# pyscf/pyscf

Hardware: NVIDIA H100
Metric: J/K Fock-build wall-s/iter (lower is better)
Workload: dtype f64

## Files before the change

### pyscf_b200/csrc/b200jk.cu

```cuda
#include "host_common.hpp"
#include "jk_classes.cuh"

namespace {

void ensure_workspace(b200jk_handle h, int n_dm)
{
    if ((size_t)n_dm <= h->ws_ndm) return;
    for (double** p : {&h->d_dm_sph, &h->d_out_sph, &h->d_dmj, &h->d_dmk, &h->d_vj, &h->d_vk}) { dev_free(*p); *p = nullptr; }
    size_t ns2 = (size_t)h->nsph * h->nsph, nc2 = (size_t)h->ncart * h->ncart;
    h->d_dm_sph = (double*)dev_alloc(ns2 * n_dm * 8);
    h->d_out_sph = (double*)dev_alloc(ns2 * n_dm * 8 * 2);
    h->d_dmj = (double*)dev_alloc(nc2 * n_dm * 8);
    h->d_dmk = (double*)dev_alloc(nc2 * n_dm * 8 * 2);
    h->d_vj = (double*)dev_alloc(nc2 * n_dm * 8);
    h->d_vk = (double*)dev_alloc(nc2 * n_dm * 8 * 2);
    h->ws_ndm = n_dm;
}

}

extern "C" const char* b200jk_version(void)
{
#ifdef B200JK_EMULATE
    return "b200jk 0.1 (CPU SIMT emulation — tests only)";
// ... 640 lines not shown
        d2h(w, dw, (size_t)count * n * 8, st);
#ifndef B200JK_EMULATE
        CK(cudaStreamSynchronize(st));
#endif
    } catch (std::exception& e) { set_err(h, e.what()); rc = 2; }
    for (void* p : tmp) dev_free(p);
    return rc;
}

extern "C" int b200jk_get_dm_cond_test(b200jk_handle h, double* dmc, int32_t* ao_off, int nsh)
{
    if (!h) return 1;
    try {
        if (!dmc || nsh != h->nsh) throw std::runtime_error("b200jk_get_dm_cond_test: nsh must be the number of device shells");
        if (!h->ws_ndm) throw std::runtime_error("b200jk_get_dm_cond_test: no b200jk_direct_jk call yet");
#ifndef B200JK_EMULATE
        CK(cudaSetDevice(h->device));
#endif
        d2h(dmc, h->d_dmc, (size_t)nsh * nsh * 8);
        dev_sync();
        if (ao_off)
            for (int i = 0; i < nsh; i++) ao_off[i] = h->sh[i].sph_off;
    } catch (std::exception& e) { set_err(h, e.what()); return 2; }
    return 0;
}

extern "C" int b200jk_get_stats(b200jk_handle h, b200jk_stats* out)
{
    if (!h || !out) return 1;
    *out = h->stats;
    return 0;
}

#ifndef B200JK_HAVE_DF
extern "C" int b200jk_df_build(b200jk_handle h, const int32_t*, int, const int32_t*, int, const double*, int, double, double)
{ set_err(h, "density-fitting path not built into this library"); return 3; }
extern "C" int b200jk_df_jk(b200jk_handle h, const double*, int, int, const double*, int, int, double*, double*)
{ set_err(h, "density-fitting path not built into this library"); return 3; }
extern "C" int b200jk_df_naux(b200jk_handle h, int*)
{ set_err(h, "density-fitting path not built into this library"); return 3; }
#endif
```

### pyscf_b200/csrc/jk_block.cuh

```cuda
#pragma once
#include "jk_core.cuh"

namespace b200jk {

constexpr int KCH_MAX = 512;
#ifndef B2_CTA_THREADS
#define B2_CTA_THREADS 192
#endif
#ifndef B2_SMEM_CAP
#define B2_SMEM_CAP 0
#endif

struct KParams {
    const ShellPair* bra_pairs; int nbra;
    const ShellPair* ket_pairs; int nket;
    int same_class;
    const PrimPair* prims;
    RysTables tb;
    double omega, tol;
    const double* dmc; int nsh;
    const double* dmj; const double* dmk;
    double* vj; double* vk;
    int n, n_dm_j, n_dm_k;
    int kchunk;
    int bra_nprim_max, ket_nprim_max;
    int shard_rank, shard_world;
    int pslice;
    unsigned long long* counters;
};

constexpr int pow2ceil(int x) { int p = 1; while (p < x) p *= 2; return p; }

#ifndef B2_PPW
#define B2_PPW 0
#endif

constexpr bool class_prefers_ppw(int li, int lj, int lk, int ll)
{
    return (li == 2 && lj == 2 && lk == 1 && ll == 1) || (li == 3 && lj == 3 && lk == 2 && ll == 0) || (li == 3 && lj == 2 && lk == 2 && ll == 0) ||
           (li == 2 && lj == 2 && lk == 2 && ll == 1) || (li == 2 && lj == 2 && lk == 2 && ll == 0) || (li == 3 && lj == 2 && lk == 1 && ll == 1);
}
template <class C>
struct GroupCfg {
    static constexpr int G = C::G;
    static constexpr bool PPW = (B2_PPW > 0 || (B2_PPW == 0 && class_prefers_ppw(C::LI, C::LJ, C::LK, C::LL))) && C::NP > 1 && C::NKL <= 32 && C::NP <= 8;
    static constexpr int GP = G <= 32 ? G : ((G + 31) / 32) * 32;
    static constexpr int GW = PPW ? C::NP : (GP + 31) / 32;
    static constexpr int TG = GW * 32;
    static constexpr int QPG = PPW ? 32 / C::NKL : (GP <= 32 ? 32 / GP : 1);
    static constexpr int NG0 = B2_CTA_THREADS / TG;
    static constexpr int NG1 = NG0 < 1 ? 1 : (NG0 > 8 ? 8 : NG0);
    static constexpr int NG2 = (NG1 * QPG > 64) ? ((64 / QPG) < 1 ? 1 : 64 / QPG) : NG1;
    static constexpr int NGC = B2_SMEM_CAP > 0 ? (int)(B2_SMEM_CAP / (QPG * sizeof(SlotSmem<C>))) : NG2;
    static constexpr int NG = NGC < 1 ? 1 : (NGC < NG2 ? NGC : NG2);
    static constexpr int NT = NG * TG;
    static constexpr int NSLOT = NG * QPG;
    static B2_HD bool decode(int lt, int& sl, int& g)
    {
        const int w = lt / 32, l = lt % 32;
        sl = l / C::NKL;
        g = w * C::NKL + l % C::NKL;
        if (sl >= QPG) { sl = 0; g = 0; return false; }
        return true;
    }
};

template <class C>
struct BlockSmem {
    SlotSmem<C> slot[GroupCfg<C>::NSLOT];
    BraInfo bra;
    PrimPair bprim[MAX_PRIM_PER_PAIR];
    unsigned long long mbar_bra;
    int klist[KCH_MAX];
    int nk;
    int next;
    int gbase[GroupCfg<C>::NG];
};

template <class C>
struct LaneCtx {
    ThreadCtx<C> t;
    double jij[C::NV];
    int grp, lt, slot, valid;
    int ibp, ikp;
    int sr;
};

#if defined(__CUDA_ARCH__)
#define B2_ALL_THREADS(tid) { const int tid = threadIdx.x;
#define B2_END }
#define B2_SYNC() __syncthreads()
#define B2_GROUP_LANES(lt) { const int lt = threadIdx.x % GroupCfg<C>::TG;
#define B2_CTX(tid) ctx
template <class C>
__device__ __forceinline__ void group_sync(int grp)
{
    if constexpr (GroupCfg<C>::GW == 1) __syncwarp();
    else asm volatile("bar.sync %0, %1;" ::"r"(grp + 1), "n"(GroupCfg<C>::TG) : "memory");
}
#else
#define B2_ALL_THREADS(tid) for (int tid = 0; tid < GroupCfg<C>::NT; tid++) {
#define B2_END }
#define B2_SYNC()
#define B2_GROUP_LANES(lt) for (int lt = 0; lt < GroupCfg<C>::TG; lt++) {
#define B2_CTX(tid) ctxs[tid]
template <class C>
inline void group_sync(int) {}
#endif

#if defined(__CUDA_ARCH__)
__device__ __forceinline__ void bulk_g2s(void* dst, const void* src, unsigned bytes, unsigned long long* bar)
{
    unsigned d = (unsigned)__cvta_generic_to_shared(dst), b = (unsigned)__cvta_generic_to_shared(bar);
    asm volatile("fence.proxy.async.shared::cta;" ::: "memory");
    asm volatile("mbarrier.arrive.expect_tx.shared::cta.b64 _, [%0], %1;" ::"r"(b), "r"(bytes) : "memory");
    asm volatile("cp.async.bulk.shared::cluster.global.mbarrier::complete_tx::bytes [%0], [%1], %2, [%3];"
                 ::"r"(d), "l"(src), "r"(bytes), "r"(b) : "memory");
}
__device__ __forceinline__ void bulk_wait(unsigned long long* bar, unsigned parity)
{
    unsigned b = (unsigned)__cvta_generic_to_shared(bar), ok;
    do {
        asm volatile("{\n\t.reg .pred p;\n\tmbarrier.try_wait.parity.shared::cta.b64 p, [%1], %2;\n\tselp.u32 %0, 1, 0, p;\n\t}\n"
                     : "=r"(ok) : "r"(b), "r"(parity) : "memory");
    } while (!ok);
}
#endif

template <class C, bool SR>
#ifdef __CUDACC__
__device__ __forceinline__
#else
inline
// ... 116 lines not shown

        for (int ip = 0; ip < npmax; ip++) {
            B2_GROUP_LANES(lt)
                LaneCtx<C>& L = B2_CTX(tid0 + lt);
                if (L.valid) {
                    SlotSmem<C>& s = sm.slot[L.slot];
                    if (s.active && L.ibp < nbp)
                        phase_roots<C>(s, L.t.g, sm.bprim[L.ibp], load_prim(P.prims + s.prim_off_k + L.ikp), P.tb,
                                       sr_op ? (L.sr ? -P.omega : 0.0) : P.omega, (sr_op && L.sr) ? -1.0 : 1.0);
                }
            B2_END
            group_sync<C>(grp);
            B2_GROUP_LANES(lt)
                LaneCtx<C>& L = B2_CTX(tid0 + lt);
                if (L.valid) {
                    SlotSmem<C>& s = sm.slot[L.slot];
                    if (s.active && L.ibp < nbp) phase_vrr<C>(s, L.t.g);
                }
            B2_END
            group_sync<C>(grp);
            B2_GROUP_LANES(lt)
                LaneCtx<C>& L = B2_CTX(tid0 + lt);
                if (L.valid) {
                    SlotSmem<C>& s = sm.slot[L.slot];
                    if (s.active && L.ibp < nbp) {
                        phase_accumulate<C>(s, L.t, sm.bra.ABx, sm.bra.ABy, sm.bra.ABz);
                        if (sr_op && !L.sr) L.sr = 1;
                        else { L.sr = 0; if (++L.ikp == s.nprim_k) { L.ikp = 0; L.ibp++; } }
                    }
                }
            B2_END
        }
        }
        B2_GROUP_LANES(lt)
            LaneCtx<C>& L = B2_CTX(tid0 + lt);
            if (L.valid) {
                SlotSmem<C>& s = sm.slot[L.slot];
                if (s.active) {
                    if (P.vj) phase_digest<C>(s, L.t, sm.bra.i0, sm.bra.j0, P.n, P.n_dm_j, P.dmj, nullptr, P.vj, nullptr,
                                              P.n_dm_j == 1 ? L.jij : nullptr);
                    if (P.vk) phase_digest<C>(s, L.t, sm.bra.i0, sm.bra.j0, P.n, P.n_dm_k, nullptr, P.dmk, nullptr, P.vk, nullptr);
                }
            }
        B2_END
        group_sync<C>(grp);
    }
}

template <class C, bool SR>
#ifdef __CUDACC__
__device__ __forceinline__
#else
inline
#endif
void jk_block(const KParams& P, int bx, int by, BlockSmem<C>& sm)
{
    using GC = GroupCfg<C>;
    const ShellPair& bpair = P.bra_pairs[bx];
    const int kmax = P.same_class ? (bx + 1) : P.nket;
    const int kbeg = by * P.kchunk;
    const int kend = (kbeg + P.kchunk < kmax) ? kbeg + P.kchunk : kmax;
    if (kbeg >= kend) return;
#if defined(__CUDA_ARCH__)
    LaneCtx<C> ctx;
#else
    LaneCtx<C>* ctxs = new LaneCtx<C>[GC::NT];
#endif

    B2_ALL_THREADS(tid)
        LaneCtx<C>& L = B2_CTX(tid);
        L.grp = tid / GC::TG;
        L.lt = tid % GC::TG;
        if constexpr (GC::PPW) {
            int sl, g;
            L.valid = GC::decode(L.lt, sl, g);
            L.slot = L.grp * GC::QPG + sl;
            thread_decode<C>(L.t, g);
// ... 33 lines not shown
        const int send = (sub + KCH_MAX < kend) ? sub + KCH_MAX : kend;
        if (sub > kbeg) {
            B2_SYNC();
            B2_ALL_THREADS(tid)
                if (tid == 0) { sm.nk = 0; sm.next = 0; }
            B2_END
            B2_SYNC();
        }
        B2_ALL_THREADS(tid)
            for (int kk = sub + tid; kk < send; kk += GC::NT) {
                const ShellPair& kp = P.ket_pairs[kk];
                bool keep = keep_quartet(bpair.q, kp.q, bpair.ish, bpair.jsh, kp.ish, kp.jsh, P.dmc, P.nsh, P.tol,
                                         P.vj != nullptr, P.vk != nullptr);
                if (keep) {
#if defined(__CUDA_ARCH__)
                    int pos = atomicAdd(&sm.nk, 1);
#else
                    int pos = sm.nk++;
#endif
                    sm.klist[pos] = kk;
                }
            }
        B2_END
        B2_SYNC();
        const int nk = sm.nk;
#if defined(__CUDA_ARCH__)
        if (P.counters && threadIdx.x == 0) {
            atomicAdd(&P.counters[0], (unsigned long long)nk);
            atomicAdd(&P.counters[1], (unsigned long long)(send - sub - nk));
        }
        group_proc<C, SR>(P, sm, threadIdx.x / GC::TG, nk, bx, ctx);
#else
        if (P.counters) { P.counters[0] += nk; P.counters[1] += send - sub - nk; }
        for (int grp = 0; grp < GC::NG; grp++) group_proc<C, SR>(P, sm, grp, nk, bx, ctxs);
#endif
    }

    if (P.vj && P.n_dm_j == 1) {
        B2_ALL_THREADS(tid)
            LaneCtx<C>& L = B2_CTX(tid);
            if (L.valid) {
                const int b0 = L.t.p * C::NJP;
                B2_UNROLL
                for (int bb = 0; bb < C::NJP; bb++) {
                    B2_UNROLL
                    for (int a = 0; a < C::NI; a++) {
                        double val = L.jij[bb * C::NI + a];
                        if (val != 0.0) red_add(&P.vj[(size_t)(sm.bra.i0 + a) * P.n + (sm.bra.j0 + b0 + bb)], val);
                    }
                }
            }
        B2_END
    }
#if !defined(__CUDA_ARCH__)
    delete[] ctxs;
#endif
}

}
```

### pyscf_b200/csrc/jk_core.cuh

```cuda
#pragma once
#include <math.h>
#include <stdint.h>

#ifdef __CUDACC__
#define B2_HD __host__ __device__ __forceinline__
#define B2_UNROLL _Pragma("unroll")
#define B2_NOUNROLL _Pragma("unroll 1")
#else
#define B2_HD inline __attribute__((always_inline))
#define B2_UNROLL
#define B2_NOUNROLL
#endif

namespace b200jk {

#ifndef __CUDACC__
inline double rsqrt(double x) { return 1.0 / sqrt(x); }
#endif

constexpr int LMAX = 4;
constexpr int RYS_NMAX = 9, RYS_DEG = 7, RYS_NINT = 320;
constexpr double RYS_H = 0.3125, RYS_XMAX = 100.0;
constexpr int RYS_ROW = 2 * (RYS_DEG + 1);
constexpr double PI_25_2 = 34.98683665524972497;
// ... 356 lines not shown

template <class C, int P>
struct PartDispatch {
    static B2_HD void run(int p, double* v, const double* gx, const double* gy, const double* gz)
    {
        if (p == P) accumulate_part<C, P>(v, gx, gy, gz);
        else PartDispatch<C, P + 1>::run(p, v, gx, gy, gz);
    }
};
template <class C>
struct PartDispatch<C, C::NP> {
    static B2_HD void run(int, double*, const double*, const double*, const double*) {}
};

template <class C>
B2_HD void phase_accumulate(const SlotSmem<C>& s, ThreadCtx<C>& t, double ABx, double ABy, double ABz, int b = 0)
{
    for (int r = 0; r < C::NR; r++) {
        double gx[C::NI1 * C::NJ1], gy[C::NI1 * C::NJ1], gz[C::NI1 * C::NJ1];
        hrr_dir<C>(s.H[b][0][r], t.kx, t.lx, ABx, gx);
        hrr_dir<C>(s.H[b][1][r], t.ky, t.ly, ABy, gy);
        hrr_dir<C>(s.H[b][2][r], t.kz, t.lz, ABz, gz);
        PartDispatch<C, 0>::run(t.p, t.v, gx, gy, gz);
    }
}

#ifdef __CUDA_ARCH__
#ifdef B2_EXPERIMENT_NORED
__device__ __forceinline__ void red_add(double* addr, double val) { if (val == 1.2345678e301) atomicAdd(addr, val); }
#else
__device__ __forceinline__ void red_add(double* addr, double val) { atomicAdd(addr, val); }
#endif
#else
inline void red_add(double* addr, double val) { *addr += val; }
#endif

#if defined(__CUDA_ARCH__)
#define B2_LDG(p) __ldg(p)
#else
#define B2_LDG(p) (*(p))
#endif

template <class C>
B2_HD void phase_digest(const SlotSmem<C>& s, const ThreadCtx<C>& t, int i0, int j0, int n, int n_dm,
                        const double* dmj, const double* dmk, double* vj, double* vk, double* jacc)
{
    const double f = s.fac;
    const int kc = s.k0 + t.c, ld = s.l0 + t.d;
    const int b0 = t.p * C::NJP;
    const size_t n2 = (size_t)n * n;
    for (int idm = 0; idm < n_dm; idm++) {
        if (vj) {
            const double* D = dmj + idm * n2;
            double* J = vj + idm * n2;
            double dkl = 2.0 * f * B2_LDG(&D[(size_t)kc * n + ld]);
            double jkl = 0.0;
            B2_UNROLL
            for (int bb = 0; bb < C::NJP; bb++) {
                B2_UNROLL
                for (int a = 0; a < C::NI; a++) {
                    double val = t.v[bb * C::NI + a];
                    size_t ij = (size_t)(i0 + a) * n + (j0 + b0 + bb);
                    jkl += val * B2_LDG(&D[ij]);
                    if (jacc) jacc[bb * C::NI + a] += val * dkl;
                    else red_add(&J[ij], val * dkl);
                }
            }
// ... 9 lines not shown
            for (int a = 0; a < C::NI; a++) {
                kik[a] = 0.0; kil[a] = 0.0;
                dik[a] = B2_LDG(&D[(size_t)(i0 + a) * n + kc]);
                dil[a] = B2_LDG(&D[(size_t)(i0 + a) * n + ld]);
            }
            B2_UNROLL
            for (int bb = 0; bb < C::NJP; bb++) {
                int jb = j0 + b0 + bb;
                double djl = B2_LDG(&D[(size_t)jb * n + ld]), djk = B2_LDG(&D[(size_t)jb * n + kc]);
                double sjk = 0.0, sjl = 0.0;
                B2_UNROLL
                for (int a = 0; a < C::NI; a++) {
                    double val = t.v[bb * C::NI + a];
                    kik[a] += val * djl;
                    kil[a] += val * djk;
                    sjk += val * dil[a];
                    sjl += val * dik[a];
                }
                kjk[bb] = sjk; kjl[bb] = sjl;
            }
            B2_UNROLL
            for (int a = 0; a < C::NI; a++) {
                red_add(&K[(size_t)(i0 + a) * n + kc], f * kik[a]);
                red_add(&K[(size_t)(i0 + a) * n + ld], f * kil[a]);
            }
            B2_UNROLL
            for (int bb = 0; bb < C::NJP; bb++) {
                int jb = j0 + b0 + bb;
                red_add(&K[(size_t)jb * n + kc], f * kjk[bb]);
                red_add(&K[(size_t)jb * n + ld], f * kjl[bb]);
            }
        }
    }
}

B2_HD bool keep_quartet(double qij, double qkl, int ish, int jsh, int ksh, int lsh, const double* dmc, int nsh,
                        double tol, bool do_j, bool do_k)
{
    double qq = qij * qkl;
    if (!(qq > tol)) return false;
    double dmin = tol / qq;
    bool keep = false;
    if (do_j) keep = (4.0 * dmc[ish * nsh + jsh] > dmin) || (4.0 * dmc[ksh * nsh + lsh] > dmin);
    if (do_k && !keep)
        keep = (dmc[jsh * nsh + ksh] > dmin) || (dmc[jsh * nsh + lsh] > dmin) || (dmc[ish * nsh + ksh] > dmin) ||
               (dmc[ish * nsh + lsh] > dmin);
    return keep;
}

B2_HD double schwarz_pair(int la, int lb, const ShellPair& sp, const PrimPair* prims, const RysTables& tb, double omega)
{
    const int L = la + lb;
    const int nr = L + 1;
    const int na = ncart(la), nb = ncart(lb);
    double acc[ncart(LMAX) * ncart(LMAX)];
    for (int e = 0; e < na * nb; e++) acc[e] = 0.0;
    double AB[3] = {sp.ABx, sp.ABy, sp.ABz};
    for (int ip = 0; ip < sp.nprim; ip++)
        for (int kp = 0; kp < sp.nprim; kp++) {
            const PrimPair& bp = prims[sp.prim_off + ip];
            const PrimPair& kq = prims[sp.prim_off + kp];
            double p = bp.p, q = kq.p, pq = p + q, ipq = 1.0 / pq;
            double PQ[3] = {bp.Px - kq.Px, bp.Py - kq.Py, bp.Pz - kq.Pz};
            double PA[3] = {bp.PAx, bp.PAy, bp.PAz}, QC[3] = {kq.PAx, kq.PAy, kq.PAz};
            double rho = p * q * ipq;
            double x = rho * (PQ[0] * PQ[0] + PQ[1] * PQ[1] + PQ[2] * PQ[2]);
// ... 157 lines not shown
```

### pyscf_b200/csrc/jk_classes.cuh

```cuda
#pragma once
#include <cstdlib>
#include <stdexcept>
#include "jk_tpq.cuh"

namespace b200jk {

constexpr int lane_eff_permille(int g) { return g <= 32 ? (32 / g) * g * 1000 / 32 : g * 1000 / (((g + 31) / 32) * 32); }

#ifndef B2_NVMAX
#define B2_NVMAX 30
#endif
#ifndef B2_WANT_CTAS
#define B2_WANT_CTAS 2
#endif
#ifndef B2_PBMAX
#define B2_PBMAX 1
#endif
#ifndef B2_CARVEOUT
#define B2_CARVEOUT -1
#endif

constexpr int choose_np(int ni, int nj, int nkl)
{
    int nab = ni * nj;
    int best = 0, best_eff = -1;
    for (int np = 1; np <= nj; np++) {
        if (nj % np != 0 || nab / np > B2_NVMAX) continue;
        if (best && nab / np < 15) break;
        if (nkl * np > 512) break;
        int eff = lane_eff_permille(nkl * np);
        if (eff > best_eff + 60) { best = np; best_eff = eff; }
    }
    return best ? best : nj;
}

constexpr int choose_pb(int g, int nr, int h_bytes, int nslot)
// ... 26 lines not shown
    static const long want_env = getenv("B200JK_WANT_CTAS") ? atol(getenv("B200JK_WANT_CTAS")) : 0;
    long want_ctas = device_sm_count() * (want_env > 0 ? want_env : B2_WANT_CTAS);
    long ny = (want_ctas + nbra - 1) / nbra;
    long kc = (nket + ny - 1) / ny;
    if (kc < unit) kc = unit;
    if (kc > cap) kc = cap;
    return (int)kc;
}

inline int kets_cap(int round1_cap)
{
    static const bool old_cap = getenv("B200JK_KETS_CAP") && atoi(getenv("B200JK_KETS_CAP")) == 1;
    return old_cap ? round1_cap : (1 << 30);
}

template <int LI, int LJ, int LK, int LL>
struct ClassCfg {
    static constexpr int NP = choose_np(ncart(LI), ncart(LJ), ncart(LK) * ncart(LL));
    using C1 = QClass<LI, LJ, LK, LL, NP>;
    static constexpr int PB = (LI + LJ >= 6) ? 1 : choose_pb(C1::G, C1::NR, 3 * C1::NR * C1::HSP * 8, GroupCfg<C1>::NSLOT);
    using C = QClass<LI, LJ, LK, LL, NP, PB>;
    using GC = GroupCfg<C>;
    static constexpr int NT = GC::NT;
    static constexpr int KC0 = GC::NSLOT * 8;
    static constexpr int KCHUNK = KC0 > KCH_MAX ? KCH_MAX : (KC0 < 64 ? 64 : KC0);
};

#ifndef B200JK_EMULATE
template <class C, bool SR>
__global__ void __launch_bounds__(TpqCfg<C>::NT) jk_tpq_kernel(const KParams P)
{
    const int bx = blockIdx.x * P.shard_world + P.shard_rank;
    if (bx < P.nbra) tpq_block<C, SR>(P, bx, blockIdx.y, blockIdx.z);
}
#ifndef B2_MINB
#define B2_MINB -1
#endif
constexpr bool class_caps_registers(int li, int lj, int lk, int ll)
{
    if (B2_MINB == 0) return false;
    if (B2_MINB > 0) return true;
    if (li == 3 && lj == 1) return false;
    if (li == 3 && lj == 2 && lk == 1 && ll == 0) return false;
    if (li == 3 && lj == 2 && lk == 3 && ll == 1) return false;
    if (li == 2 && lj == 0 && lk == 1 && ll == 1) return false;
    if (li == 1 && lj == 1 && lk == 1 && ll == 1) return false;
    return true;
}
template <class C, bool SR>
__global__ void __launch_bounds__(GroupCfg<C>::NT) jk_class_kernel(const KParams P)
{
    extern __shared__ __align__(16) unsigned char smraw[];
    BlockSmem<C>& sm = *reinterpret_cast<BlockSmem<C>*>(smraw);
    const int bx = blockIdx.x * P.shard_world + P.shard_rank;
    if (bx < P.nbra) jk_block<C, SR>(P, bx, blockIdx.y, sm);
}
template <class C, bool SR>
__global__ void __launch_bounds__(GroupCfg<C>::NT, 2) jk_class_kernel_2cta(const KParams P)
{
    extern __shared__ __align__(16) unsigned char smraw[];
    BlockSmem<C>& sm = *reinterpret_cast<BlockSmem<C>*>(smraw);
    const int bx = blockIdx.x * P.shard_world + P.shard_rank;
    if (bx < P.nbra) jk_block<C, SR>(P, bx, blockIdx.y, sm);
}
#endif

// ... 53 lines not shown
    cudaError_t e = cudaGetLastError();
    if (e != cudaSuccess) throw std::runtime_error(std::string("jk_class_kernel launch: ") + cudaGetErrorString(e));
}
#endif

template <int LI, int LJ, int LK, int LL>
void launch_one(KParams P, b2_stream_t st)
{
    using Cfg = ClassCfg<LI, LJ, LK, LL>;
    using C = typename Cfg::C;
    if constexpr (TpqCfg<C>::eligible) {
        {
            static const int ps_env = getenv("B200JK_TPQ_PSLICE") ? atoi(getenv("B200JK_TPQ_PSLICE")) : 0;
            P.pslice = ps_env > 0 ? ps_env : TpqCfg<C>::PSLICE;
        }
        const int nbx = (P.nbra + P.shard_world - 1) / P.shard_world;
        P.kchunk = pick_kchunk(nbx, P.nket, TpqCfg<C>::NT, kets_cap(TpqCfg<C>::KCHUNK));
        int ny = (P.nket + P.kchunk - 1) / P.kchunk;
#ifndef B200JK_EMULATE
        dim3 grid(nbx, ny, (P.bra_nprim_max + P.pslice - 1) / P.pslice);
        if (P.omega < 0.0) jk_tpq_kernel<C, true><<<grid, TpqCfg<C>::NT, 0, st>>>(P);
        else jk_tpq_kernel<C, false><<<grid, TpqCfg<C>::NT, 0, st>>>(P);
        cudaError_t e = cudaGetLastError();
        if (e != cudaSuccess) throw std::runtime_error(std::string("jk_tpq_kernel launch: ") + cudaGetErrorString(e));
#else
        (void)st;
        for (int bx = P.shard_rank; bx < P.nbra; bx += P.shard_world)
            for (int by = 0; by < ny; by++)
                for (int bz = 0; bz * P.pslice < P.bra_nprim_max; bz++) {
                    if (P.omega < 0.0) tpq_block<C, true>(P, bx, by, bz);
                    else tpq_block<C, false>(P, bx, by, bz);
                }
#endif
        return;
    }
    const int nbx = (P.nbra + P.shard_world - 1) / P.shard_world;
    P.kchunk = pick_kchunk(nbx, P.nket, Cfg::GC::NSLOT, kets_cap(KCH_MAX));
    int ny = (P.nket + P.kchunk - 1) / P.kchunk;
#ifndef B200JK_EMULATE
    size_t smem = sizeof(BlockSmem<C>);
    dim3 grid(nbx, ny);
    if (P.omega < 0.0) launch_block_kernel<C, true>(P, grid, Cfg::NT, smem, st);
    else launch_block_kernel<C, false>(P, grid, Cfg::NT, smem, st);
#else
    (void)st;
    BlockSmem<C>* sm = new BlockSmem<C>();
    for (int bx = P.shard_rank; bx < P.nbra; bx += P.shard_world)
        for (int by = 0; by < ny; by++) {
            if (P.omega < 0.0) jk_block<C, true>(P, bx, by, *sm);
            else jk_block<C, false>(P, bx, by, *sm);
        }
    delete sm;
#endif
}

constexpr int B2_LAUNCH_INFO_N = 9;
template <int LI, int LJ, int LK, int LL>
void info_one(int* out)
{
    using Cfg = ClassCfg<LI, LJ, LK, LL>;
    using C = typename Cfg::C;
    for (int i = 0; i < B2_LAUNCH_INFO_N; i++) out[i] = -1;
    const void* kern = nullptr;
    size_t smem = 0;
    if constexpr (TpqCfg<C>::eligible) {
        out[0] = 0; out[1] = TpqCfg<C>::NT;
#ifndef B200JK_EMULATE
        kern = (const void*)jk_tpq_kernel<C, false>;
#endif
    } else {
        out[0] = 1; out[1] = Cfg::NT; smem = sizeof(BlockSmem<C>);
#ifndef B200JK_EMULATE
        kern = (const void*)block_kernel<C, false>(out[6]);
#endif
    }
    out[2] = (int)smem;
#ifndef B200JK_EMULATE
    cudaFuncAttributes fa;
    b2_check(cudaFuncGetAttributes(&fa, kern), "cudaFuncGetAttributes");
    out[3] = fa.numRegs;
    out[4] = (int)fa.localSizeBytes;
    b2_check(cudaOccupancyMaxActiveBlocksPerMultiprocessor(&out[5], kern, out[1], smem), "cudaOccupancyMaxActiveBlocksPerMultiprocessor");
    b2_check(cudaOccupancyMaxActiveBlocksPerMultiprocessor(&out[7], kern, out[1], 0), "cudaOccupancyMaxActiveBlocksPerMultiprocessor");
#else
    (void)kern;
#endif
}

#define B2_PAIR_CASES(X) \
    X(0, 0, 0) X(1, 1, 0) X(2, 1, 1) X(3, 2, 0) X(4, 2, 1) X(5, 2, 2) X(6, 3, 0) X(7, 3, 1) X(8, 3, 2) X(9, 3, 3)

inline bool tpq_class(int la, int lb, int lc, int ld)
{
    int nout = ncart(la) * ncart(lb) * ncart(lc) * ncart(ld);
    int nr = (la + lb + lc + ld) / 2 + 1;
    return nout <= 36 && nr <= 3 && choose_np(ncart(la), ncart(lb), ncart(lc) * ncart(ld)) == 1;
}

constexpr bool use_swapped(int hi, int lo)
{
    return (hi == 6 && lo == 4) || (hi == 7 && lo == 4) || (hi == 6 && lo == 2) || (hi == 7 && lo == 5);
// ... 74 lines not shown
```

Before: 0.02501.

## Stage J/K digest partials in shared memory and reduce before atomics for selected classes

For a hardcoded list of angular-momentum classes, each lane writes its K (and J kl) partial sums into the slot's reused H scratch in shared memory. A group-wide reduction then sums across the lanes that target the same output element and issues one atomic per output, replacing one atomic per lane. This is meant to cut global atomic traffic and contention in the digest phase. The cost is extra group syncs, multiple passes when the scratch cannot hold all entries, and more shared-memory work. It also adds emulator-only counters for digest atomics.

```diff
diff --git a/pyscf_b200/csrc/b200jk.cu b/pyscf_b200/csrc/b200jk.cu
--- a/pyscf_b200/csrc/b200jk.cu
+++ b/pyscf_b200/csrc/b200jk.cu
@@ -696,6 +696,18 @@
     return 0;
 }
 
+#ifdef B200JK_EMULATE
+extern "C" int b200jk_emu_digest_counts(unsigned long long* out, int reset)
+{
+    for (int c = 0; c < LMAX * LMAX * LMAX * LMAX; c++) {
+        unsigned long long* e = emu_digest_counts(c / (LMAX * LMAX * LMAX), c / (LMAX * LMAX) % LMAX, c / LMAX % LMAX, c % LMAX);
+        if (out) { out[2 * c] = e[0]; out[2 * c + 1] = e[1]; }
+        if (reset) e[0] = e[1] = 0;
+    }
+    return 0;
+}
+#endif
+
 #ifndef B200JK_HAVE_DF
 extern "C" int b200jk_df_build(b200jk_handle h, const int32_t*, int, const int32_t*, int, const double*, int, double, double)
 { set_err(h, "density-fitting path not built into this library"); return 3; }
diff --git a/pyscf_b200/csrc/jk_block.cuh b/pyscf_b200/csrc/jk_block.cuh
--- a/pyscf_b200/csrc/jk_block.cuh
+++ b/pyscf_b200/csrc/jk_block.cuh
@@ -39,6 +39,14 @@
 {
     return (li == 2 && lj == 2 && lk == 1 && ll == 1) || (li == 3 && lj == 3 && lk == 2 && ll == 0) || (li == 3 && lj == 2 && lk == 2 && ll == 0) ||
            (li == 2 && lj == 2 && lk == 2 && ll == 1) || (li == 2 && lj == 2 && lk == 2 && ll == 0) || (li == 3 && lj == 2 && lk == 1 && ll == 1);
+}
+constexpr bool class_stages_digest(int li, int lj, int lk, int ll)
+{
+    constexpr int T[16][4] = {{2, 1, 3, 1}, {1, 1, 3, 0}, {2, 1, 3, 0}, {2, 2, 2, 0}, {2, 2, 1, 0}, {2, 1, 2, 0}, {2, 1, 1, 1}, {3, 2, 2, 1},
+                              {3, 2, 2, 0}, {3, 2, 1, 1}, {3, 2, 1, 0}, {3, 3, 2, 0}, {3, 1, 3, 0}, {3, 1, 1, 1}, {3, 0, 2, 0}, {3, 0, 3, 0}};
+    for (const auto& c : T)
+        if (c[0] == li && c[1] == lj && c[2] == lk && c[3] == ll) return true;
+    return false;
 }
 template <class C>
 struct GroupCfg {
@@ -99,6 +107,11 @@
     else asm volatile("bar.sync %0, %1;" ::"r"(grp + 1), "n"(GroupCfg<C>::TG) : "memory");
 }
 #else
+inline unsigned long long* emu_digest_counts(int li, int lj, int lk, int ll)
+{
+    static unsigned long long tab[LMAX * LMAX * LMAX * LMAX][2];
+    return tab[((li * LMAX + lj) * LMAX + lk) * LMAX + ll];
+}
 #define B2_ALL_THREADS(tid) for (int tid = 0; tid < GroupCfg<C>::NT; tid++) {
 #define B2_END }
 #define B2_SYNC()
@@ -281,6 +294,35 @@
             B2_END
         }
         }
+        if constexpr (class_stages_digest(C::LI, C::LJ, C::LK, C::LL)) {
+        using DC = DigestCfg<C>;
+        const size_t n2 = (size_t)P.n * P.n;
+        const int ndm_j = P.vj ? P.n_dm_j : 0, ndm_k = P.vk ? P.n_dm_k : 0;
+        const int ndm = ndm_j > ndm_k ? ndm_j : ndm_k;
+        for (int idm = 0; idm < ndm; idm++) {
+            const bool dj = idm < ndm_j, dk = idm < ndm_k;
+            const int elo = dk ? 0 : DC::NEK, ehi = dj ? DC::NE : DC::NEK;
+            for (int lo = elo; lo < ehi; lo += DC::EPP) {
+                const int hi = (lo + DC::EPP < ehi) ? lo + DC::EPP : ehi;
+                group_sync<C>(grp);
+                B2_GROUP_LANES(lt)
+                    LaneCtx<C>& L = B2_CTX(tid0 + lt);
+                    if (L.valid) {
+                        SlotSmem<C>& s = sm.slot[L.slot];
+                        if (s.active)
+                            digest_stage<C>(s, L.t, sm.bra.i0, sm.bra.j0, P.n, dj ? P.dmj + idm * n2 : nullptr,
+                                            dk ? P.dmk + idm * n2 : nullptr, dj ? P.vj + idm * n2 : nullptr,
+                                            P.n_dm_j == 1 ? L.jij : nullptr, lo, hi, &s.H[0][0][0][0]);
+                    }
+                B2_END
+                group_sync<C>(grp);
+                B2_GROUP_LANES(lt)
+                    digest_reduce<C, GC::TG, GC::QPG>(&sm.slot[grp * GC::QPG], lt, lo, hi, sm.bra.i0, sm.bra.j0, P.n,
+                                                      dj ? P.vj + idm * n2 : nullptr, dk ? P.vk + idm * n2 : nullptr);
+                B2_END
+            }
+        }
+        } else {
         B2_GROUP_LANES(lt)
             LaneCtx<C>& L = B2_CTX(tid0 + lt);
             if (L.valid) {
@@ -292,6 +334,7 @@
                 }
             }
         B2_END
+        }
         group_sync<C>(grp);
     }
 }
@@ -391,7 +434,10 @@
         group_proc<C, SR>(P, sm, threadIdx.x / GC::TG, nk, bx, ctx);
 #else
         if (P.counters) { P.counters[0] += nk; P.counters[1] += send - sub - nk; }
+        const unsigned long long red0 = emu_red_count();
         for (int grp = 0; grp < GC::NG; grp++) group_proc<C, SR>(P, sm, grp, nk, bx, ctxs);
+        unsigned long long* dc = emu_digest_counts(C::LI, C::LJ, C::LK, C::LL);
+        dc[0] += nk; dc[1] += emu_red_count() - red0;
 #endif
     }
 
diff --git a/pyscf_b200/csrc/jk_core.cuh b/pyscf_b200/csrc/jk_core.cuh
--- a/pyscf_b200/csrc/jk_core.cuh
+++ b/pyscf_b200/csrc/jk_core.cuh
@@ -412,7 +412,8 @@
 __device__ __forceinline__ void red_add(double* addr, double val) { atomicAdd(addr, val); }
 #endif
 #else
-inline void red_add(double* addr, double val) { *addr += val; }
+inline unsigned long long& emu_red_count() { static unsigned long long n = 0; return n; }
+inline void red_add(double* addr, double val) { *addr += val; emu_red_count()++; }
 #endif
 
 #if defined(__CUDA_ARCH__)
@@ -488,6 +489,157 @@
             }
         }
     }
+}
+
+template <class C>
+struct DigestCfg {
+    static constexpr int NEK = 2 * (C::NI + C::NJP);
+    static constexpr int NE = NEK + 1;
+    static constexpr int HCAP = C::PB * 3 * C::NR * C::HSP;
+    static constexpr int EPP = HCAP / C::G;
+    static_assert(EPP >= 1, "a quartet's lanes must fit one partial each into the slot's H");
+};
+
+template <class C>
+B2_HD void stage_put(double* scr, int lo, int hi, int e, int idx, double x)
+{
+    if (e >= lo && e < hi) scr[(e - lo) * C::G + idx] = x;
+}
+
+template <class C>
+B2_HD void digest_stage(const SlotSmem<C>& s, const ThreadCtx<C>& t, int i0, int j0, int n, const double* Dj, const double* Dk,
+                        double* J, double* jacc, int lo, int hi, double* scr)
+{
+    const int kc = s.k0 + t.c, ld = s.l0 + t.d;
+    const int b0 = t.p * C::NJP;
+    const int gc = t.p * C::NKL + t.d * C::NK + t.c, gd = t.p * C::NKL + t.c * C::NL + t.d;
+    constexpr int NEK = DigestCfg<C>::NEK;
+    if (Dk && lo < NEK) {
+        double kjk[C::NJP], kjl[C::NJP];
+        double kik[C::NI], kil[C::NI];
+        double dik[C::NI], dil[C::NI];
+        B2_UNROLL
+        for (int a = 0; a < C::NI; a++) {
+            kik[a] = 0.0; kil[a] = 0.0;
+            dik[a] = B2_LDG(&Dk[(size_t)(i0 + a) * n + kc]);
+            dil[a] = B2_LDG(&Dk[(size_t)(i0 + a) * n + ld]);
+        }
+        B2_UNROLL
+        for (int bb = 0; bb < C::NJP; bb++) {
+            int jb = j0 + b0 + bb;
+            double djl = B2_LDG(&Dk[(size_t)jb * n + ld]), djk = B2_LDG(&Dk[(size_t)jb * n + kc]);
+            double sjk = 0.0, sjl = 0.0;
+            B2_UNROLL
+            for (int a = 0; a < C::NI; a++) {
+                double val = t.v[bb * C::NI + a];
+                kik[a] += val * djl;
+                kil[a] += val * djk;
+                sjk += val * dil[a];
+                sjl += val * dik[a];
+            }
+            kjk[bb] = sjk; kjl[bb] = sjl;
+        }
+        B2_UNROLL
+        for (int a = 0; a < C::NI; a++) {
+            stage_put<C>(scr, lo, hi, a, gc, kik[a]);
+            stage_put<C>(scr, lo, hi, C::NI + a, gd, kil[a]);
+        }
+        B2_UNROLL
+        for (int bb = 0; bb < C::NJP; bb++) {
+            stage_put<C>(scr, lo, hi, 2 * C::NI + bb, gc, kjk[bb]);
+            stage_put<C>(scr, lo, hi, 2 * C::NI + C::NJP + bb, gd, kjl[bb]);
+        }
+    }
+    if (Dj && lo <= NEK && NEK < hi) {
+        double dkl = 2.0 * s.fac * B2_LDG(&Dj[(size_t)kc * n + ld]);
+        double jkl = 0.0;
+        B2_UNROLL
+        for (int bb = 0; bb < C::NJP; bb++) {
+            B2_UNROLL
+            for (int a = 0; a < C::NI; a++) {
+                double val = t.v[bb * C::NI + a];
+                size_t ij = (size_t)(i0 + a) * n + (j0 + b0 + bb);
+                jkl += val * B2_LDG(&Dj[ij]);
+                if (jacc) jacc[bb * C::NI + a] += val * dkl;
+                else red_add(&J[ij], val * dkl);
+            }
+        }
+        scr[(NEK - lo) * C::G + gd] = jkl;
+    }
+}
+
+template <class C, int SEC> struct DigestSec;
+template <class C> struct DigestSec<C, 0> {
+    static constexpr int E0 = 0, E1 = C::NI, NOUT = C::NK, N2 = C::NP, S2 = C::NKL, N1 = C::NL, S1 = C::NK;
+    static constexpr double SCALE = 1.0;
+    static B2_HD int base(int o) { return o; }
+    static B2_HD void dest(int e, int o, const SlotSmem<C>& s, int i0, int, int& r, int& c) { r = i0 + e; c = s.k0 + o; }
+};
+template <class C> struct DigestSec<C, 1> {
+    static constexpr int E0 = C::NI, E1 = 2 * C::NI, NOUT = C::NL, N2 = C::NP, S2 = C::NKL, N1 = C::NK, S1 = C::NL;
+    static constexpr double SCALE = 1.0;
+    static B2_HD int base(int o) { return o; }
+    static B2_HD void dest(int e, int o, const SlotSmem<C>& s, int i0, int, int& r, int& c) { r = i0 + e - E0; c = s.l0 + o; }
+};
+template <class C> struct DigestSec<C, 2> {
+    static constexpr int E0 = 2 * C::NI, E1 = 2 * C::NI + C::NJP, NOUT = C::NP * C::NK, N2 = 1, S2 = 0, N1 = C::NL, S1 = C::NK;
+    static constexpr double SCALE = 1.0;
+    static B2_HD int base(int o) { return (o / C::NK) * C::NKL + o % C::NK; }
+    static B2_HD void dest(int e, int o, const SlotSmem<C>& s, int, int j0, int& r, int& c)
+    {
+        r = j0 + (o / C::NK) * C::NJP + e - E0; c = s.k0 + o % C::NK;
+    }
+};
+template <class C> struct DigestSec<C, 3> {
+    static constexpr int E0 = 2 * C::NI + C::NJP, E1 = DigestCfg<C>::NEK, NOUT = C::NP * C::NL, N2 = 1, S2 = 0, N1 = C::NK, S1 = C::NL;
+    static constexpr double SCALE = 1.0;
+    static B2_HD int base(int o) { return (o / C::NL) * C::NKL + o % C::NL; }
+    static B2_HD void dest(int e, int o, const SlotSmem<C>& s, int, int j0, int& r, int& c)
+    {
+        r = j0 + (o / C::NL) * C::NJP + e - E0; c = s.l0 + o % C::NL;
+    }
+};
+template <class C> struct DigestSec<C, 4> {
+    static constexpr int E0 = DigestCfg<C>::NEK, E1 = E0 + 1, NOUT = C::NKL, N2 = 1, S2 = 0, N1 = C::NP, S1 = C::NKL;
+    static constexpr double SCALE = 2.0;
+    static B2_HD int base(int o) { return o; }
+    static B2_HD void dest(int, int o, const SlotSmem<C>& s, int, int, int& r, int& c) { r = s.k0 + o / C::NL; c = s.l0 + o % C::NL; }
+};
+
+template <class C, int TG, int QPG, int SEC>
+B2_HD int digest_reduce_sec(const SlotSmem<C>* slots, int lt, int off, int lo, int hi, int i0, int j0, int n, double* out)
+{
+    using S = DigestSec<C, SEC>;
+    const int e0 = S::E0 > lo ? S::E0 : lo, e1 = S::E1 < hi ? S::E1 : hi;
+    if (!out || e1 <= e0) return off;
+    const int cnt = (e1 - e0) * QPG * S::NOUT;
+    for (int task = ((lt - off) % TG + TG) % TG; task < cnt; task += TG) {
+        const int o = task % S::NOUT, rq = task / S::NOUT, q = rq % QPG, e = e0 + rq / QPG;
+        const SlotSmem<C>& s = slots[q];
+        if (!s.active) continue;
+        const double* x = &s.H[0][0][0][0] + (e - lo) * C::G + S::base(o);
+        double sum = 0.0;
+        B2_UNROLL
+        for (int i2 = 0; i2 < S::N2; i2++) {
+            B2_UNROLL
+            for (int i1 = 0; i1 < S::N1; i1++) sum += x[i2 * S::S2 + i1 * S::S1];
+        }
+        int r, c;
+        S::dest(e, o, s, i0, j0, r, c);
+        red_add(&out[(size_t)r * n + c], S::SCALE * s.fac * sum);
+    }
+    return off + cnt;
+}
+
+template <class C, int TG, int QPG>
+B2_HD void digest_reduce(const SlotSmem<C>* slots, int lt, int lo, int hi, int i0, int j0, int n, double* J, double* K)
+{
+    int off = 0;
+    off = digest_reduce_sec<C, TG, QPG, 0>(slots, lt, off, lo, hi, i0, j0, n, K);
+    off = digest_reduce_sec<C, TG, QPG, 1>(slots, lt, off, lo, hi, i0, j0, n, K);
+    off = digest_reduce_sec<C, TG, QPG, 2>(slots, lt, off, lo, hi, i0, j0, n, K);
+    off = digest_reduce_sec<C, TG, QPG, 3>(slots, lt, off, lo, hi, i0, j0, n, K);
+    digest_reduce_sec<C, TG, QPG, 4>(slots, lt, off, lo, hi, i0, j0, n, J);
 }
 
 B2_HD bool keep_quartet(double qij, double qkl, int ish, int jsh, int ksh, int lsh, const double* dmc, int nsh,
```

Result: faster. 0.02434, median of 6 (-2.7%).

## Add sub-warp quartet kernel splitting ket components across lanes for mid-L classes

Applied to the files above, without the earlier changes.

Adds a new 'swq' kernel path in which a few lanes (2 to 8) cooperate on one shell quartet. Each lane computes the Rys VRR for all ket components and then selects its own subset of kl components, keeping its accumulators in registers. It applies to eight mid-angular-momentum classes that previously used the shared-memory block kernel, aiming to avoid shared-memory staging and raise occupancy. The cost is redundant VRR work across lanes and more per-lane atomics in the digest step.

```diff
diff --git a/pyscf_b200/csrc/jk_classes.cuh b/pyscf_b200/csrc/jk_classes.cuh
--- a/pyscf_b200/csrc/jk_classes.cuh
+++ b/pyscf_b200/csrc/jk_classes.cuh
@@ -1,7 +1,7 @@
 #pragma once
 #include <cstdlib>
 #include <stdexcept>
-#include "jk_tpq.cuh"
+#include "jk_swq.cuh"
 
 namespace b200jk {
 
@@ -94,6 +94,12 @@
 {
     const int bx = blockIdx.x * P.shard_world + P.shard_rank;
     if (bx < P.nbra) tpq_block<C, SR>(P, bx, blockIdx.y, blockIdx.z);
+}
+template <class C, bool SR>
+__global__ void __launch_bounds__(SwqCfg<C>::NT) jk_swq_kernel(const KParams P)
+{
+    const int bx = blockIdx.x * P.shard_world + P.shard_rank;
+    if (bx < P.nbra) swq_block<C, SR>(P, bx, blockIdx.y, blockIdx.z);
 }
 #ifndef B2_MINB
 #define B2_MINB -1
@@ -213,26 +219,47 @@
                     else tpq_block<C, false>(P, bx, by, bz);
                 }
 #endif
-        return;
-    }
-    const int nbx = (P.nbra + P.shard_world - 1) / P.shard_world;
-    P.kchunk = pick_kchunk(nbx, P.nket, Cfg::GC::NSLOT, kets_cap(KCH_MAX));
-    int ny = (P.nket + P.kchunk - 1) / P.kchunk;
-#ifndef B200JK_EMULATE
-    size_t smem = sizeof(BlockSmem<C>);
-    dim3 grid(nbx, ny);
-    if (P.omega < 0.0) launch_block_kernel<C, true>(P, grid, Cfg::NT, smem, st);
-    else launch_block_kernel<C, false>(P, grid, Cfg::NT, smem, st);
-#else
-    (void)st;
-    BlockSmem<C>* sm = new BlockSmem<C>();
-    for (int bx = P.shard_rank; bx < P.nbra; bx += P.shard_world)
-        for (int by = 0; by < ny; by++) {
-            if (P.omega < 0.0) jk_block<C, true>(P, bx, by, *sm);
-            else jk_block<C, false>(P, bx, by, *sm);
-        }
-    delete sm;
-#endif
+    } else if constexpr (SwqCfg<C>::eligible) {
+        using W = SwqCfg<C>;
+        P.pslice = W::PSLICE;
+        const int nbx = (P.nbra + P.shard_world - 1) / P.shard_world;
+        P.kchunk = pick_kchunk(nbx, P.nket, W::NSLOT, kets_cap(W::KCHUNK));
+        int ny = (P.nket + P.kchunk - 1) / P.kchunk;
+#ifndef B200JK_EMULATE
+        dim3 grid(nbx, ny, (P.bra_nprim_max + P.pslice - 1) / P.pslice);
+        if (P.omega < 0.0) jk_swq_kernel<C, true><<<grid, W::NT, 0, st>>>(P);
+        else jk_swq_kernel<C, false><<<grid, W::NT, 0, st>>>(P);
+        cudaError_t e = cudaGetLastError();
+        if (e != cudaSuccess) throw std::runtime_error(std::string("jk_swq_kernel launch: ") + cudaGetErrorString(e));
+#else
+        (void)st;
+        for (int bx = P.shard_rank; bx < P.nbra; bx += P.shard_world)
+            for (int by = 0; by < ny; by++)
+                for (int bz = 0; bz * P.pslice < P.bra_nprim_max; bz++) {
+                    if (P.omega < 0.0) swq_block<C, true>(P, bx, by, bz);
+                    else swq_block<C, false>(P, bx, by, bz);
+                }
+#endif
+    } else {
+        const int nbx = (P.nbra + P.shard_world - 1) / P.shard_world;
+        P.kchunk = pick_kchunk(nbx, P.nket, Cfg::GC::NSLOT, kets_cap(KCH_MAX));
+        int ny = (P.nket + P.kchunk - 1) / P.kchunk;
+#ifndef B200JK_EMULATE
+        size_t smem = sizeof(BlockSmem<C>);
+        dim3 grid(nbx, ny);
+        if (P.omega < 0.0) launch_block_kernel<C, true>(P, grid, Cfg::NT, smem, st);
+        else launch_block_kernel<C, false>(P, grid, Cfg::NT, smem, st);
+#else
+        (void)st;
+        BlockSmem<C>* sm = new BlockSmem<C>();
+        for (int bx = P.shard_rank; bx < P.nbra; bx += P.shard_world)
+            for (int by = 0; by < ny; by++) {
+                if (P.omega < 0.0) jk_block<C, true>(P, bx, by, *sm);
+                else jk_block<C, false>(P, bx, by, *sm);
+            }
+        delete sm;
+#endif
+    }
 }
 
 constexpr int B2_LAUNCH_INFO_N = 9;
@@ -248,6 +275,11 @@
         out[0] = 0; out[1] = TpqCfg<C>::NT;
 #ifndef B200JK_EMULATE
         kern = (const void*)jk_tpq_kernel<C, false>;
+#endif
+    } else if constexpr (SwqCfg<C>::eligible) {
+        out[0] = 2; out[1] = SwqCfg<C>::NT;
+#ifndef B200JK_EMULATE
+        kern = (const void*)jk_swq_kernel<C, false>;
 #endif
     } else {
         out[0] = 1; out[1] = Cfg::NT; smem = sizeof(BlockSmem<C>);
diff --git a/pyscf_b200/csrc/jk_swq.cuh b/pyscf_b200/csrc/jk_swq.cuh
--- /dev/null
+++ b/pyscf_b200/csrc/jk_swq.cuh
@@ -0,0 +1,339 @@
+#pragma once
+#include "jk_tpq.cuh"
+
+namespace b200jk {
+
+constexpr int SWQ_NACC = 36;
+
+constexpr int swq_lanes(int nab, int nkl)
+{
+    for (int t = 2; t <= 8; t *= 2)
+        if ((nkl + t - 1) / t * nab <= SWQ_NACC) return t;
+    return 0;
+}
+
+constexpr bool swq_class(int li, int lj, int lk, int ll)
+{
+    return (li == 2 && lj == 1 && lk == 1 && ll == 0) ||
+           (li == 2 && lj == 0 && lk == 1 && ll == 1) ||
+           (li == 2 && lj == 1 && lk == 2 && ll == 0) ||
+           (li == 3 && lj == 0 && lk == 2 && ll == 0) ||
+           (li == 3 && lj == 1 && lk == 1 && ll == 0) ||
+           (li == 2 && lj == 2 && lk == 1 && ll == 0) ||
+           (li == 1 && lj == 1 && lk == 3 && ll == 0) ||
+           (li == 1 && lj == 1 && lk == 1 && ll == 1);
+}
+
+template <class C>
+struct SwqCfg {
+    static constexpr int NAB = C::NI * C::NJ, NKL = C::NKL;
+    static constexpr int T = swq_lanes(NAB, NKL);
+    static constexpr int S = T ? (NKL + T - 1) / T : 1;
+    static constexpr bool eligible = swq_class(C::LI, C::LJ, C::LK, C::LL) && T > 0 && C::NR <= 3;
+    static constexpr int NT = B2_TPQ_NT;
+    static constexpr int NSLOT = T ? NT / T : 1;
+    static constexpr int PSLICE = B2_TPQ_PSLICE;
+    static constexpr int KCHUNK = B2_TPQ_KCHUNK;
+    static constexpr int GI = C::LI + 1, GKL = (C::LK + 1) * (C::LL + 1);
+};
+
+template <class C>
+B2_HD void swq_vrr(double c00, double c0p, double b00, double b10, double b01, double i00, double CD, double* K)
+{
+    double I[C::NB1][C::NT1];
+    I[0][0] = i00;
+    if (C::LB > 0) {
+        I[1][0] = c00 * i00;
+        B2_UNROLL
+        for (int n = 1; n < C::LB; n++) I[n + 1][0] = c00 * I[n][0] + n * b10 * I[n - 1][0];
+    }
+    B2_UNROLL
+    for (int m = 0; m < C::LT; m++) {
+        B2_UNROLL
+        for (int n = 0; n <= C::LB; n++) {
+            double val = c0p * I[n][m];
+            if (m > 0) val += m * b01 * I[n][m - 1];
+            if (n > 0) val += n * b00 * I[n - 1][m];
+            I[n][m + 1] = val;
+        }
+    }
+    B2_UNROLL
+    for (int l = 0; l <= C::LL; l++) {
+        if (l > 0) {
+            B2_UNROLL
+            for (int n = 0; n <= C::LB; n++) {
+                B2_UNROLL
+                for (int m = 0; m <= C::LT - l; m++) I[n][m] = I[n][m + 1] + CD * I[n][m];
+            }
+        }
+        B2_UNROLL
+        for (int k = 0; k <= C::LK; k++) {
+            B2_UNROLL
+            for (int n = 0; n <= C::LB; n++) K[(l * (C::LK + 1) + k) * C::NB1 + n] = I[n][k];
+        }
+    }
+}
+
+template <class C>
+B2_HD void swq_pick(const double* K, int kl, double AB, double* g)
+{
+    using W = SwqCfg<C>;
+    double X[C::NB1];
+    B2_UNROLL
+    for (int n = 0; n <= C::LB; n++) X[n] = K[n];
+    B2_UNROLL
+    for (int e = 1; e < W::GKL; e++) {
+        const bool m = (e == kl);
+        B2_UNROLL
+        for (int n = 0; n <= C::LB; n++) X[n] = m ? K[e * C::NB1 + n] : X[n];
+    }
+    B2_UNROLL
+    for (int i = 0; i <= C::LI; i++) g[i] = X[i];
+    B2_UNROLL
+    for (int j = 1; j <= C::LJ; j++) {
+        B2_UNROLL
+        for (int n = 0; n <= C::LB - j; n++) X[n] = X[n + 1] + AB * X[n];
+        B2_UNROLL
+        for (int i = 0; i <= C::LI; i++) g[j * W::GI + i] = X[i];
+    }
+}
+
+struct SwqLane {
+    int kx[8], ky[8], kz[8];
+};
+
+template <class C, bool SR>
+B2_HD void swq_eri(const KParams& P, const ShellPair& bp, const ShellPair& kp, int ib0, int ib1, const SwqLane& ln, double* v)
+{
+    using W = SwqCfg<C>;
+    B2_UNROLL
+    for (int e = 0; e < W::S * W::NAB; e++) v[e] = 0.0;
+    for (int ik = 0; ik < kp.nprim; ik++) {
+        const PrimPair k = load_prim(P.prims + kp.prim_off + ik);
+        for (int ib = ib0; ib < ib1; ib++) {
+            const PrimPair b = load_prim(P.prims + bp.prim_off + ib);
+            double p = b.p, q = k.p;
+            double PQx = b.Px - k.Px, PQy = b.Py - k.Py, PQz = b.Pz - k.Pz;
+            double pq = p + q;
+            double rs = rsqrt(pq);
+            double ipq = rs * rs;
+            double rho = p * q * ipq;
+            double x = rho * (PQx * PQx + PQy * PQy + PQz * PQz);
+            const double x0 = x, pref0 = b.cc * k.cc * rs;
+            double hip = 0.5 / p, hiq = 0.5 / q;
+            if (C::LB == 0) hip = 0.0;
+            if (C::LT == 0) hiq = 0.0;
+            constexpr int nsr = SR ? 2 : 1;
+            B2_NOUNROLL
+            for (int sr = 0; sr < nsr; sr++) {
+            double pref = pref0;
+            double theta = 1.0;
+            const double om = (nsr == 2) ? (sr ? -P.omega : 0.0) : P.omega;
+            x = x0;
+            if (om > 0.0) {
+                theta = om * om / (om * om + rho);
+                x *= theta;
+                pref *= sqrt(theta);
+            }
+            if (sr) pref = -pref;
+            B2_NOUNROLL
+            for (int r = 0; r < C::NR; r++) {
+                double u, w;
+                rys_root(P.tb, C::NR, r, x, u, w);
+                u *= theta; w *= pref;
+                double b00 = 0.5 * u * ipq;
+                double b10 = (1.0 - u * q * ipq) * hip;
+                double b01 = (1.0 - u * p * ipq) * hiq;
+                double uq = u * q * ipq, up = u * p * ipq;
+                double Kx[W::GKL * C::NB1], Ky[W::GKL * C::NB1], Kz[W::GKL * C::NB1];
+                swq_vrr<C>(b.PAx - uq * PQx, k.PAx + up * PQx, b00, b10, b01, 1.0, kp.ABx, Kx);
+                swq_vrr<C>(b.PAy - uq * PQy, k.PAy + up * PQy, b00, b10, b01, 1.0, kp.ABy, Ky);
+                swq_vrr<C>(b.PAz - uq * PQz, k.PAz + up * PQz, b00, b10, b01, w, kp.ABz, Kz);
+                B2_UNROLL
+                for (int s = 0; s < W::S; s++) {
+                    double gx[W::GI * (C::LJ + 1)], gy[W::GI * (C::LJ + 1)], gz[W::GI * (C::LJ + 1)];
+                    swq_pick<C>(Kx, ln.kx[s], bp.ABx, gx);
+                    swq_pick<C>(Ky, ln.ky[s], bp.ABy, gy);
+                    swq_pick<C>(Kz, ln.kz[s], bp.ABz, gz);
+                    B2_UNROLL
+                    for (int bb = 0; bb < C::NJ; bb++) {
+                        B2_UNROLL
+                        for (int a = 0; a < C::NI; a++) {
+                            const int ix = cart_px(C::LI, a), iy = cart_py(C::LI, a), iz = C::LI - ix - iy;
+                            const int jx = cart_px(C::LJ, bb), jy = cart_py(C::LJ, bb), jz = C::LJ - jx - jy;
+                            v[s * W::NAB + bb * C::NI + a] +=
+                                gx[jx * W::GI + ix] * gy[jy * W::GI + iy] * gz[jz * W::GI + iz];
+                        }
+                    }
+                }
+            }
+            }
+        }
+    }
+}
+
+template <class C>
+B2_HD void swq_digest(const KParams& P, const double* v, double f, int i0, int j0, int kc, int ld, bool one_j, double* jij)
+{
+    using W = SwqCfg<C>;
+    const int n = P.n;
+    const size_t n2 = (size_t)n * n;
+    if (P.vj) {
+        for (int idm = 0; idm < P.n_dm_j; idm++) {
+            const double* D = P.dmj + idm * n2;
+            double* J = P.vj + idm * n2;
+            const double dkl = 2.0 * f * B2_LDG(&D[(size_t)kc * n + ld]);
+            double jkl = 0.0;
+            B2_UNROLL
+            for (int e = 0; e < W::NAB; e++) {
+                const size_t ij = (size_t)(i0 + e % C::NI) * n + j0 + e / C::NI;
+                jkl += v[e] * B2_LDG(&D[ij]);
+                if (one_j) jij[e] += v[e] * dkl;
+                else red_add(&J[ij], v[e] * dkl);
+            }
+            red_add(&J[(size_t)kc * n + ld], 2.0 * f * jkl);
+        }
+    }
+    if (P.vk) {
+        for (int idm = 0; idm < P.n_dm_k; idm++) {
+            const double* D = P.dmk + idm * n2;
+            double* K = P.vk + idm * n2;
+            double kik[C::NI], kil[C::NI], dik[C::NI], dil[C::NI], kjk[C::NJ], kjl[C::NJ], djk[C::NJ], djl[C::NJ];
+            B2_UNROLL
+            for (int a = 0; a < C::NI; a++) {
+                kik[a] = 0.0; kil[a] = 0.0;
+                dik[a] = B2_LDG(&D[(size_t)(i0 + a) * n + kc]);
+                dil[a] = B2_LDG(&D[(size_t)(i0 + a) * n + ld]);
+            }
+            B2_UNROLL
+            for (int bb = 0; bb < C::NJ; bb++) {
+                djk[bb] = B2_LDG(&D[(size_t)(j0 + bb) * n + kc]);
+                djl[bb] = B2_LDG(&D[(size_t)(j0 + bb) * n + ld]);
+            }
+            B2_UNROLL
+            for (int bb = 0; bb < C::NJ; bb++) {
+                double sjk = 0.0, sjl = 0.0;
+                B2_UNROLL
+                for (int a = 0; a < C::NI; a++) {
+                    const double val = v[bb * C::NI + a];
+                    kik[a] += val * djl[bb];
+                    kil[a] += val * djk[bb];
+                    sjk += val * dil[a];
+                    sjl += val * dik[a];
+                }
+                kjk[bb] = sjk; kjl[bb] = sjl;
+            }
+            B2_UNROLL
+            for (int a = 0; a < C::NI; a++) {
+                red_add(&K[(size_t)(i0 + a) * n + kc], f * kik[a]);
+                red_add(&K[(size_t)(i0 + a) * n + ld], f * kil[a]);
+            }
+            B2_UNROLL
+            for (int bb = 0; bb < C::NJ; bb++) {
+                red_add(&K[(size_t)(j0 + bb) * n + kc], f * kjk[bb]);
+                red_add(&K[(size_t)(j0 + bb) * n + ld], f * kjl[bb]);
+            }
+        }
+    }
+}
+
+template <class C, bool SR>
+#ifdef __CUDACC__
+__device__ __forceinline__
+#else
+inline
+#endif
+void swq_block(const KParams& P, int bx, int by, int bz)
+{
+    using W = SwqCfg<C>;
+    static_assert(W::T > 0 && W::S <= 8 && 32 % W::T == 0, "sub-warp layout");
+    const ShellPair bpair = P.bra_pairs[bx];
+    const int kmax = P.same_class ? (bx + 1) : P.nket;
+    const int kbeg = by * P.kchunk;
+    const int kend = (kbeg + P.kchunk < kmax) ? kbeg + P.kchunk : kmax;
+    if (kbeg >= kend) return;
+    const int ib0 = bz * P.pslice;
+    const int ib1 = (ib0 + P.pslice < bpair.nprim) ? ib0 + P.pslice : bpair.nprim;
+    if (ib0 >= ib1) return;
+#if defined(__CUDA_ARCH__)
+    {
+        const int tid = threadIdx.x;
+#else
+    double jsum[W::NAB];
+    for (int e = 0; e < W::NAB; e++) jsum[e] = 0.0;
+    unsigned long long ncomp = 0, nskip = 0;
+    for (int tid = 0; tid < W::NT; tid++) {
+#endif
+        const int slot = tid / W::T, t = tid % W::T;
+        SwqLane ln;
+        int cof[W::S], dof[W::S];
+        B2_UNROLL
+        for (int s = 0; s < W::S; s++) {
+            int cd = t + s * W::T;
+            if (cd >= W::NKL) cd = 0;
+            const int c = cd % C::NK, d = cd / C::NK;
+            cof[s] = c; dof[s] = d;
+            ln.kx[s] = cart_px(C::LL, d) * (C::LK + 1) + cart_px(C::LK, c);
+            ln.ky[s] = cart_py(C::LL, d) * (C::LK + 1) + cart_py(C::LK, c);
+            ln.kz[s] = cart_pz(C::LL, d) * (C::LK + 1) + cart_pz(C::LK, c);
+        }
+        double jij[W::NAB];
+        const bool one_j = P.vj && P.n_dm_j == 1;
+        B2_UNROLL
+        for (int e = 0; e < W::NAB; e++) jij[e] = 0.0;
+        int mine = 0, skipped = 0;
+        for (int kk = kbeg + slot; kk < kend; kk += W::NSLOT) {
+            const ShellPair kp = load_pair(P.ket_pairs + kk);
+            if (!keep_quartet(bpair.q, kp.q, bpair.ish, bpair.jsh, kp.ish, kp.jsh, P.dmc, P.nsh, P.tol, P.vj != nullptr,
+                              P.vk != nullptr)) {
+                if (bz == 0 && t == 0) skipped++;
+                continue;
+            }
+            if (bz == 0 && t == 0) mine++;
+            double f = 1.0;
+            if (bpair.same) f *= 0.5;
+            if (kp.same) f *= 0.5;
+            if (P.same_class && kk == bx) f *= 0.5;
+            double v[W::S * W::NAB];
+            swq_eri<C, SR>(P, bpair, kp, ib0, ib1, ln, v);
+            B2_UNROLL
+            for (int s = 0; s < W::S; s++)
+                if (t + s * W::T < W::NKL)
+                    swq_digest<C>(P, v + s * W::NAB, f, bpair.i0, bpair.j0, kp.i0 + cof[s], kp.j0 + dof[s], one_j, jij);
+        }
+#if defined(__CUDA_ARCH__)
+        if (one_j) {
+            B2_UNROLL
+            for (int e = 0; e < W::NAB; e++) {
+                double val = jij[e];
+                B2_UNROLL
+                for (int o = 16; o > 0; o >>= 1) val += __shfl_xor_sync(0xffffffffu, val, o);
+                if ((tid & 31) == 0 && val != 0.0)
+                    atomicAdd(&P.vj[(size_t)(bpair.i0 + e % C::NI) * P.n + bpair.j0 + e / C::NI], val);
+            }
+        }
+        if (P.counters) {
+            int tot = mine;
+            B2_UNROLL
+            for (int o = 16; o > 0; o >>= 1) tot += __shfl_xor_sync(0xffffffffu, tot, o);
+            int sk = skipped;
+            B2_UNROLL
+            for (int o = 16; o > 0; o >>= 1) sk += __shfl_xor_sync(0xffffffffu, sk, o);
+            if ((tid & 31) == 0) {
+                atomicAdd(&P.counters[0], (unsigned long long)tot);
+                atomicAdd(&P.counters[1], (unsigned long long)sk);
+            }
+        }
+    }
+#else
+        for (int e = 0; e < W::NAB; e++) jsum[e] += jij[e];
+        ncomp += mine;
+        nskip += skipped;
+    }
+    if (P.vj && P.n_dm_j == 1)
+        for (int e = 0; e < W::NAB; e++) P.vj[(size_t)(bpair.i0 + e % C::NI) * P.n + bpair.j0 + e / C::NI] += jsum[e];
+    if (P.counters) { P.counters[0] += ncomp; P.counters[1] += nskip; }
+#endif
+}
+
+}
```

Measured after the change: 0.02511 before, 0.02361 after, median of 6. 1.06x faster.
